# hellolijj/gpu-topology-on-k8s

Measured on AMD Instinct MI355X. Metric: RCCL all-reduce bus GB/s on scheduler-chosen k-GPU subset, k=1/2/4/8, higher is better.
Workload: dtype bf16

## Files before the change

csrc/common/stream_copy.h:

```cpp
#pragma once
#include <hip/hip_runtime.h>

#include <algorithm>
#include <cstddef>

namespace gtk {

typedef unsigned int u32x4 __attribute__((ext_vector_type(4)));

constexpr int kStreamBlock = 256;

template <int U>
__device__ __forceinline__ size_t stream_slices(const u32x4* __restrict__ src, u32x4* __restrict__ dst, size_t n_vec,
                                                size_t blk, size_t nblk) {
  const size_t tile = (size_t)kStreamBlock * U;
  const size_t n_tiles = n_vec / tile;
  const size_t per = (n_tiles + nblk - 1) / nblk;
  const size_t t0 = blk * per;
  const size_t t1 = std::min(n_tiles, t0 + per);
  for (size_t t = t0; t < t1; ++t) {
    const size_t base = t * tile + threadIdx.x;
    u32x4 r[U];
#pragma unroll
    for (int u = 0; u < U; ++u) r[u] = __builtin_nontemporal_load(src + base + (size_t)u * kStreamBlock);
#pragma unroll
    for (int u = 0; u < U; ++u) __builtin_nontemporal_store(r[u], dst + base + (size_t)u * kStreamBlock);
  }
  return n_tiles * tile;
}

__device__ __forceinline__ void stream_vec_tail(const u32x4* __restrict__ src, u32x4* __restrict__ dst, size_t n_vec,
                                                size_t first, size_t blk, size_t nblk) {
  for (size_t i = first + blk * kStreamBlock + threadIdx.x; i < n_vec; i += nblk * kStreamBlock) dst[i] = src[i];
}

}
```

csrc/rccl/rccl_core.h:

```cpp
#pragma once
#include <hip/hip_runtime.h>
#include <rccl/rccl.h>

#include <algorithm>
#include <cstdint>
#include <cstdlib>
#include <cstring>
#include <stdexcept>
#include <string>
#include <vector>

#include "self_copy.h"

#define RCCL_HIP_CHECK(expr)                                                                     \
  do {                                                                                           \
    hipError_t _e = (expr);                                                                      \
    if (_e != hipSuccess)                                                                        \
      throw std::runtime_error(std::string(#expr " failed: ") + hipGetErrorString(_e) + " at " + \
                               __FILE__ + ":" + std::to_string(__LINE__));                       \
  } while (0)

#define NCCL_CHECK(expr)                                                                          \
  do {                                                                                            \
    ncclResult_t _r = (expr);                                                                     \
    if (_r != ncclSuccess)                                                                        \
      throw std::runtime_error(std::string(#expr " failed: ") + ncclGetErrorString(_r) + " at " + \
                               __FILE__ + ":" + std::to_string(__LINE__));                        \
  } while (0)

namespace gtk {

inline ncclDataType_t parse_dtype(const std::string& s, size_t* elem) {
  if (s == "bf16" || s == "bfloat16") {
    *elem = 2;
    return ncclBfloat16;
  }
  if (s == "fp16" || s == "half" || s == "float16") {
    *elem = 2;
    return ncclFloat16;
  }
  if (s == "fp32" || s == "float" || s == "float32") {
    *elem = 4;
    return ncclFloat32;
  }
  throw std::invalid_argument("dtype must be bf16|fp16|fp32");
}

inline double bus_factor(int k) { return k > 1 ? 2.0 * (k - 1) / k : 0.0; }

__global__ void gtk_fill_kernel(void* buf, size_t count, int dtype_code, int rank) {
  const float scale = (float)(rank + 1);
  for (size_t i = (size_t)blockIdx.x * blockDim.x + threadIdx.x; i < count; i += (size_t)gridDim.x * blockDim.x) {
    float v = scale * (float)((i % 7) + 1);
    if (dtype_code == 0) {
      __bf16 b = (__bf16)v;
      reinterpret_cast<__bf16*>(buf)[i] = b;
    } else if (dtype_code == 1) {
      reinterpret_cast<_Float16*>(buf)[i] = (_Float16)v;
    } else {
      reinterpret_cast<float*>(buf)[i] = v;
    }
  }
}

__global__ void gtk_check_kernel(const void* buf, size_t count, int dtype_code, int nranks,
                                 unsigned long long* bad) {
  const float tri = (float)(nranks * (nranks + 1) / 2);
  unsigned long long local = 0;
  for (size_t i = (size_t)blockIdx.x * blockDim.x + threadIdx.x; i < count; i += (size_t)gridDim.x * blockDim.x) {
    float want = tri * (float)((i % 7) + 1);
    float got;
    if (dtype_code == 0)
      got = (float)reinterpret_cast<const __bf16*>(buf)[i];
    else if (dtype_code == 1)
      got = (float)reinterpret_cast<const _Float16*>(buf)[i];
    else
      got = reinterpret_cast<const float*>(buf)[i];
    local += (got != want);
  }
  if (local) atomicAdd(bad, local);
}

inline int dtype_code(ncclDataType_t t) { return t == ncclBfloat16 ? 0 : (t == ncclFloat16 ? 1 : 2); }
inline size_t elem_size(ncclDataType_t t) { return t == ncclFloat32 ? 4 : 2; }

struct RankState {
  int device = -1, rank = 0, nranks = 1;
  ncclComm_t comm = nullptr;
  hipStream_t stream = nullptr;
  void* send = nullptr;
  void* recv = nullptr;
  size_t cap_bytes = 0;
  bool self_copy = true;
  size_t self_copy_min = kSelfCopyMinBytes;
  int cus = 0, max_blocks = 0;

  void set_device() const { RCCL_HIP_CHECK(hipSetDevice(device)); }

  void configure() {
    const char* e = std::getenv("GTK_RCCL_SELF_COPY");
    self_copy = !(e && std::strcmp(e, "0") == 0);
    RCCL_HIP_CHECK(hipDeviceGetAttribute(&cus, hipDeviceAttributeMultiprocessorCount, device));
    max_blocks = std::max(1, cus) * kSelfCopyBlocksPerCU;
  }

  void ensure(size_t bytes) {
    set_device();
    if (!stream) RCCL_HIP_CHECK(hipStreamCreateWithFlags(&stream, hipStreamNonBlocking));
    if (bytes <= cap_bytes) return;
    if (send) RCCL_HIP_CHECK(hipFree(send));
    if (recv) RCCL_HIP_CHECK(hipFree(recv));
    send = recv = nullptr;
    RCCL_HIP_CHECK(hipMalloc(&send, bytes));
    RCCL_HIP_CHECK(hipMalloc(&recv, bytes));
    cap_bytes = bytes;
  }

  void fill(size_t count, ncclDataType_t t) {
    set_device();
    hipLaunchKernelGGL(gtk_fill_kernel, dim3(1024), dim3(256), 0, stream, send, count, dtype_code(t), rank);
    RCCL_HIP_CHECK(hipGetLastError());
  }

  unsigned long long check(size_t count, ncclDataType_t t, bool inplace) {
    set_device();
    unsigned long long* d_bad = nullptr;
    RCCL_HIP_CHECK(hipMalloc(&d_bad, sizeof(unsigned long long)));
    RCCL_HIP_CHECK(hipMemsetAsync(d_bad, 0, sizeof(unsigned long long), stream));
    hipLaunchKernelGGL(gtk_check_kernel, dim3(1024), dim3(256), 0, stream, inplace ? send : recv, count, dtype_code(t),
                       nranks, d_bad);
    RCCL_HIP_CHECK(hipGetLastError());
    unsigned long long bad = 0;
    RCCL_HIP_CHECK(hipMemcpyAsync(&bad, d_bad, sizeof(bad), hipMemcpyDeviceToHost, stream));
    RCCL_HIP_CHECK(hipStreamSynchronize(stream));
    RCCL_HIP_CHECK(hipFree(d_bad));
    return bad;
  }

  void allreduce(size_t count, ncclDataType_t t, bool inplace) {
    if (nranks == 1 && self_copy) {
      if (inplace) return;
      const size_t bytes = count * elem_size(t);
      if (bytes >= self_copy_min) {
        if (!max_blocks) throw std::logic_error("RankState::configure() was not called");
        hipLaunchKernelGGL(gtk_self_copy_kernel, dim3(self_copy_grid(bytes, max_blocks)), dim3(kSelfCopyBlock), 0, stream,
                           send, recv, bytes);
        RCCL_HIP_CHECK(hipGetLastError());
        return;
      }
    }
    NCCL_CHECK(ncclAllReduce(send, inplace ? send : recv, count, t, ncclSum, comm, stream));
  }

  void release() {
    if (comm) {
      (void)hipSetDevice(device);
      (void)ncclCommDestroy(comm);
      comm = nullptr;
    }
    if (send) (void)hipFree(send);
    if (recv) (void)hipFree(recv);
    send = recv = nullptr;
    cap_bytes = 0;
    if (stream) (void)hipStreamDestroy(stream);
    stream = nullptr;
  }
};

struct SweepPoint {
  size_t bytes = 0;
  size_t count = 0;
  double time_us = 0, algbw = 0, busbw = 0;
  unsigned long long wrong = 0;
};

class LocalGroup {
 public:
  explicit LocalGroup(const std::vector<int>& devs) : ranks_(devs.size()) {
    if (devs.empty()) throw std::invalid_argument("empty device list");
    std::vector<ncclComm_t> comms(devs.size());
    std::vector<int> dl(devs.begin(), devs.end());
    NCCL_CHECK(ncclCommInitAll(comms.data(), (int)devs.size(), dl.data()));
    for (size_t i = 0; i < devs.size(); ++i) {
      ranks_[i].device = devs[i];
      ranks_[i].rank = (int)i;
      ranks_[i].nranks = (int)devs.size();
      ranks_[i].comm = comms[i];
      ranks_[i].configure();
    }
  }
  ~LocalGroup() {
    for (auto& r : ranks_) r.release();
  }
  LocalGroup(const LocalGroup&) = delete;
  LocalGroup& operator=(const LocalGroup&) = delete;

  SweepPoint run(size_t bytes, const std::string& dtype, int iters, int warmup, bool inplace, bool check) {
    size_t elem = 0;
    ncclDataType_t t = parse_dtype(dtype, &elem);
    const size_t count = std::max<size_t>(1, bytes / elem);
    bytes = count * elem;
    for (auto& r : ranks_) r.ensure(bytes);
    SweepPoint p;
    p.bytes = bytes;
    p.count = count;
    if (check) {
      for (auto& r : ranks_) r.fill(count, t);
      launch_all(count, t, inplace);
      sync_all();
      for (auto& r : ranks_) p.wrong += r.check(count, t, inplace);
    }
    for (int i = 0; i < warmup; ++i) launch_all(count, t, inplace);
    sync_all();
    std::vector<hipEvent_t> e0(ranks_.size()), e1(ranks_.size());
    for (size_t i = 0; i < ranks_.size(); ++i) {
      ranks_[i].set_device();
      RCCL_HIP_CHECK(hipEventCreate(&e0[i]));
      RCCL_HIP_CHECK(hipEventCreate(&e1[i]));
      RCCL_HIP_CHECK(hipEventRecord(e0[i], ranks_[i].stream));
    }
    for (int i = 0; i < iters; ++i) launch_all(count, t, inplace);
    float worst = 0.f;
    for (size_t i = 0; i < ranks_.size(); ++i) {
      ranks_[i].set_device();
      RCCL_HIP_CHECK(hipEventRecord(e1[i], ranks_[i].stream));
    }
    for (size_t i = 0; i < ranks_.size(); ++i) {
      ranks_[i].set_device();
      RCCL_HIP_CHECK(hipEventSynchronize(e1[i]));
      float ms = 0.f;
      RCCL_HIP_CHECK(hipEventElapsedTime(&ms, e0[i], e1[i]));
      worst = std::max(worst, ms);
      (void)hipEventDestroy(e0[i]);
      (void)hipEventDestroy(e1[i]);
    }
    p.time_us = worst * 1e3 / std::max(1, iters);
    p.algbw = (double)bytes / (p.time_us * 1e-6) / 1e9;
    p.busbw = p.algbw * bus_factor((int)ranks_.size());
    return p;
  }

  size_t size() const { return ranks_.size(); }
  void set_self_copy(bool on) {
    for (auto& r : ranks_) r.self_copy = on;
  }

 private:
  void launch_all(size_t count, ncclDataType_t t, bool inplace) {
    NCCL_CHECK(ncclGroupStart());
    for (auto& r : ranks_) {
      r.set_device();
      r.allreduce(count, t, inplace);
    }
    NCCL_CHECK(ncclGroupEnd());
  }
  void sync_all() {
    for (auto& r : ranks_) {
      r.set_device();
      RCCL_HIP_CHECK(hipStreamSynchronize(r.stream));
    }
  }
  std::vector<RankState> ranks_;
};

inline std::vector<size_t> size_sweep(size_t min_bytes, size_t max_bytes, int factor) {
  std::vector<size_t> out;
  factor = std::max(2, factor);
  for (size_t b = std::max<size_t>(min_bytes, 4); b <= max_bytes; b *= (size_t)factor) {
    out.push_back(b);
    if (b > max_bytes / (size_t)factor) break;
  }
  return out;
}

}
```

csrc/rccl/rccl_module.hip:

```cpp
#include <pybind11/pybind11.h>
#include <pybind11/stl.h>

#include "rccl_core.h"

namespace py = pybind11;
using namespace gtk;

namespace {

class Comm {
 public:
  Comm(py::bytes uid, int nranks, int rank, int device, int min_ctas, int max_ctas) {
    std::string s = uid;
    if (s.size() != sizeof(ncclUniqueId)) throw std::invalid_argument("unique id must be NCCL_UNIQUE_ID_BYTES long");
    ncclUniqueId id;
    std::memcpy(&id, s.data(), sizeof(id));
    st_.device = device;
    st_.rank = rank;
    st_.nranks = nranks;
    py::gil_scoped_release nogil;
    st_.set_device();
    st_.configure();
    if (min_ctas > 0 || max_ctas > 0) {
      ncclConfig_t cfg = NCCL_CONFIG_INITIALIZER;
      if (min_ctas > 0) cfg.minCTAs = min_ctas;
      if (max_ctas > 0) cfg.maxCTAs = max_ctas;
      NCCL_CHECK(ncclCommInitRankConfig(&st_.comm, nranks, id, rank, &cfg));
    } else {
      NCCL_CHECK(ncclCommInitRank(&st_.comm, nranks, id, rank));
    }
    min_ctas_ = min_ctas;
    max_ctas_ = max_ctas;
    RCCL_HIP_CHECK(hipStreamCreateWithFlags(&st_.stream, hipStreamNonBlocking));
  }
  ~Comm() {
    drop_graph();
    st_.release();
  }

  void prepare(size_t bytes, const std::string& dtype) {
    drop_graph();
    t_ = parse_dtype(dtype, &elem_);
    count_ = std::max<size_t>(1, bytes / elem_);
    st_.ensure(count_ * elem_);
    st_.fill(count_, t_);
    RCCL_HIP_CHECK(hipStreamSynchronize(st_.stream));
  }

  void step(bool inplace) {
    if (!count_) throw std::runtime_error("prepare() first");
    st_.set_device();
    st_.allreduce(count_, t_, inplace);
  }

  void synchronize() {
    st_.set_device();
    RCCL_HIP_CHECK(hipStreamSynchronize(st_.stream));
  }

  unsigned long long check(bool inplace) {
    if (!count_) throw std::runtime_error("prepare() first");
    st_.fill(count_, t_);
    st_.allreduce(count_, t_, inplace);
    return st_.check(count_, t_, inplace);
  }

  void capture(int n, bool inplace) {
    if (!count_) throw std::runtime_error("prepare() first");
    if (n < 1) throw std::invalid_argument("capture needs n >= 1");
    drop_graph();
    st_.set_device();
    st_.allreduce(count_, t_, inplace);
    RCCL_HIP_CHECK(hipStreamSynchronize(st_.stream));
    hipGraph_t g = nullptr;
    RCCL_HIP_CHECK(hipStreamBeginCapture(st_.stream, hipStreamCaptureModeThreadLocal));
    try {
      for (int i = 0; i < n; ++i) st_.allreduce(count_, t_, inplace);
    } catch (...) {
      (void)hipStreamEndCapture(st_.stream, &g);
      if (g) (void)hipGraphDestroy(g);
      throw;
    }
    RCCL_HIP_CHECK(hipStreamEndCapture(st_.stream, &g));
    hipError_t e = hipGraphInstantiate(&exec_, g, nullptr, nullptr, 0);
    (void)hipGraphDestroy(g);
    if (e != hipSuccess) {
      exec_ = nullptr;
      throw std::runtime_error(std::string("hipGraphInstantiate failed: ") + hipGetErrorString(e));
    }
    graph_n_ = n;
  }

  void replay() {
    if (!exec_) throw std::runtime_error("capture() first");
    st_.set_device();
    RCCL_HIP_CHECK(hipGraphLaunch(exec_, st_.stream));
  }

  int graph_ops() const { return graph_n_; }

  unsigned long long verify() {
    if (!count_) throw std::runtime_error("prepare() first");
    return st_.check(count_, t_, false);
  }

  py::bytes read_result(size_t first, size_t n, bool inplace) {
    if (!count_ || !st_.send || !st_.recv) throw std::runtime_error("prepare() first");
    if (first > count_ || n > count_ - first) throw std::out_of_range("read_result: range outside the prepared buffer");
    std::string host(n * elem_, '\0');
    if (n) {
      py::gil_scoped_release nogil;
      st_.set_device();
      const char* src = static_cast<const char*>(inplace ? st_.send : st_.recv) + first * elem_;
      RCCL_HIP_CHECK(hipMemcpyAsync(&host[0], src, n * elem_, hipMemcpyDeviceToHost, st_.stream));
      RCCL_HIP_CHECK(hipStreamSynchronize(st_.stream));
    }
    return py::bytes(host);
  }

  size_t bytes() const { return count_ * elem_; }
  size_t count() const { return count_; }
  int rank() const { return st_.rank; }
  int nranks() const { return st_.nranks; }
  int device() const { return st_.device; }
  int min_ctas() const { return min_ctas_; }
  int max_ctas() const { return max_ctas_; }
  bool self_copy() const { return st_.self_copy; }
  void set_self_copy(bool on) {
    if (on != st_.self_copy) drop_graph();
    st_.self_copy = on;
  }
  size_t self_copy_min_bytes() const { return st_.self_copy_min; }
  void set_self_copy_min_bytes(size_t bytes) {
    if (bytes != st_.self_copy_min) drop_graph();
    st_.self_copy_min = bytes;
  }
  int self_copy_cus() const { return st_.cus; }
  int self_copy_max_blocks() const { return st_.max_blocks; }
  void destroy() {
    drop_graph();
    st_.release();
  }

 private:
  void drop_graph() {
    if (exec_) {
      (void)hipSetDevice(st_.device);
      (void)hipStreamSynchronize(st_.stream);
      (void)hipGraphExecDestroy(exec_);
    }
    exec_ = nullptr;
    graph_n_ = 0;
  }
  hipGraphExec_t exec_ = nullptr;
  int graph_n_ = 0;

  RankState st_;
  ncclDataType_t t_ = ncclBfloat16;
  size_t elem_ = 2, count_ = 0;
  int min_ctas_ = 0, max_ctas_ = 0;
};

py::bytes unique_id() {
  ncclUniqueId id;
  NCCL_CHECK(ncclGetUniqueId(&id));
  return py::bytes(reinterpret_cast<const char*>(&id), sizeof(id));
}

py::list local_sweep(const std::vector<int>& devs, const std::vector<size_t>& sizes, const std::string& dtype, int iters,
                     int warmup, bool inplace, bool check) {
  std::vector<SweepPoint> pts;
  {
    py::gil_scoped_release nogil;
    LocalGroup g(devs);
    for (size_t b : sizes) pts.push_back(g.run(b, dtype, iters, warmup, inplace, check));
  }
  py::list out;
  for (const auto& p : pts) {
    py::dict d;
    d["bytes"] = p.bytes;
    d["count"] = p.count;
    d["time_us"] = p.time_us;
    d["algbw_gbps"] = p.algbw;
    d["busbw_gbps"] = p.busbw;
    d["wrong"] = p.wrong;
    out.append(d);
  }
  return out;
}

int version() {
  int v = 0;
  NCCL_CHECK(ncclGetVersion(&v));
  return v;
}

}

PYBIND11_MODULE(_rccl, m) {
  m.doc() = "RCCL all-reduce placement validator (xGMI)";
  m.def("version", &version);
  m.def("unique_id", &unique_id);
  m.def("bus_factor", &bus_factor, py::arg("k"));
  m.def("size_sweep", &size_sweep, py::arg("min_bytes"), py::arg("max_bytes"), py::arg("factor") = 2);
  m.def("local_sweep", &local_sweep, py::arg("devs"), py::arg("sizes"), py::arg("dtype") = "bf16", py::arg("iters") = 20,
        py::arg("warmup") = 5, py::arg("inplace") = false, py::arg("check") = true);
  py::class_<Comm>(m, "Comm")
      .def(py::init<py::bytes, int, int, int, int, int>(), py::arg("uid"), py::arg("nranks"), py::arg("rank"),
           py::arg("device"), py::arg("min_ctas") = 0, py::arg("max_ctas") = 0)
      .def("prepare", &Comm::prepare, py::arg("bytes"), py::arg("dtype") = "bf16",
           py::call_guard<py::gil_scoped_release>())
      .def("step", &Comm::step, py::arg("inplace") = false, py::call_guard<py::gil_scoped_release>())
      .def("capture", &Comm::capture, py::arg("n"), py::arg("inplace") = false, py::call_guard<py::gil_scoped_release>())
      .def("replay", &Comm::replay, py::call_guard<py::gil_scoped_release>())
      .def_property_readonly("graph_ops", &Comm::graph_ops)
      .def("verify", &Comm::verify, py::call_guard<py::gil_scoped_release>())
      .def("synchronize", &Comm::synchronize, py::call_guard<py::gil_scoped_release>())
      .def("check", &Comm::check, py::arg("inplace") = false, py::call_guard<py::gil_scoped_release>())
      .def("destroy", &Comm::destroy, py::call_guard<py::gil_scoped_release>())
      .def("read_result", &Comm::read_result, py::arg("first"), py::arg("n"), py::arg("inplace") = false)
      .def_property_readonly("bytes", &Comm::bytes)
      .def_property_readonly("count", &Comm::count)
      .def_property_readonly("rank", &Comm::rank)
      .def_property_readonly("nranks", &Comm::nranks)
      .def_property_readonly("device", &Comm::device)
      .def_property_readonly("min_ctas", &Comm::min_ctas)
      .def_property_readonly("max_ctas", &Comm::max_ctas)
      .def_property("self_copy", &Comm::self_copy, &Comm::set_self_copy)
      .def_property("self_copy_min_bytes", &Comm::self_copy_min_bytes, &Comm::set_self_copy_min_bytes)
      .def_property_readonly("self_copy_cus", &Comm::self_copy_cus)
      .def_property_readonly("self_copy_max_blocks", &Comm::self_copy_max_blocks);
  m.attr("SELF_COPY_TILE_BYTES") = kSelfCopyTileBytes;
  m.attr("SELF_COPY_BLOCKS_PER_CU") = kSelfCopyBlocksPerCU;
  m.attr("SELF_COPY_MIN_BYTES") = kSelfCopyMinBytes;
}
```

csrc/rccl/self_copy.h:

```cpp
#pragma once
#include <hip/hip_runtime.h>

#include <algorithm>
#include <cstddef>
#include <cstdint>

#include "../common/stream_copy.h"

namespace gtk {

constexpr int kSelfCopyBlock = 256;
constexpr int kSelfCopyUnroll = 4;
constexpr int kSelfCopyBlocksPerCU = 8;
constexpr size_t kSelfCopyTileVec = (size_t)kSelfCopyBlock * kSelfCopyUnroll;
constexpr size_t kSelfCopyTileBytes = kSelfCopyTileVec * sizeof(u32x4);
static_assert(kSelfCopyBlock == kStreamBlock, "stream_copy.h indexes blocks of kStreamBlock threads");

constexpr size_t kSelfCopyMinBytes = (size_t)256 << 20;

__global__ __launch_bounds__(kSelfCopyBlock) void gtk_self_copy_kernel(const void* __restrict__ src_,
                                                                        void* __restrict__ dst_, size_t bytes) {
  const u32x4* __restrict__ src = static_cast<const u32x4*>(src_);
  u32x4* __restrict__ dst = static_cast<u32x4*>(dst_);
  const size_t n_vec = bytes / sizeof(u32x4);
  const size_t first = stream_slices<kSelfCopyUnroll>(src, dst, n_vec, blockIdx.x, gridDim.x);
  stream_vec_tail(src, dst, n_vec, first, blockIdx.x, gridDim.x);
  if (blockIdx.x == 0) {
    const size_t done = n_vec * sizeof(u32x4);
    const size_t units = (bytes - done) / sizeof(uint16_t);
    if (threadIdx.x < units) {
      const uint16_t* s = reinterpret_cast<const uint16_t*>(static_cast<const char*>(src_) + done);
      uint16_t* d = reinterpret_cast<uint16_t*>(static_cast<char*>(dst_) + done);
      d[threadIdx.x] = s[threadIdx.x];
    }
  }
}

inline unsigned self_copy_grid(size_t bytes, int max_blocks) {
  const size_t tiles = (bytes + kSelfCopyTileBytes - 1) / kSelfCopyTileBytes;
  return (unsigned)std::max<size_t>(1, std::min<size_t>(tiles, (size_t)max_blocks));
}

}
```

gpu_topology_on_k8s_amd/_native/build.py:

```python
from __future__ import annotations

import argparse
import concurrent.futures as cf
import os
import shlex
import subprocess
import sys
import sysconfig
from dataclasses import dataclass, field
from pathlib import Path
from typing import Dict, List, Optional

HERE = Path(__file__).resolve().parent
REPO = HERE.parent.parent
CSRC = REPO / "csrc"
ROCM = Path(os.environ.get("ROCM_PATH", "/opt/rocm"))
ARCH = os.environ.get("GTK_OFFLOAD_ARCH", "gfx950")
EXT = sysconfig.get_config_var("EXT_SUFFIX") or ".so"


def _py_includes() -> List[str]:
    import pybind11

    return [f"-I{sysconfig.get_paths()['include']}", f"-I{pybind11.get_include()}"]


def _torch_flags() -> List[str]:
    import torch
    from torch.utils import cpp_extension as ce

    inc = [f"-I{p}" for p in ce.include_paths()]
    libdir = str(Path(torch.__file__).parent / "lib")
    return inc + [
        "-D__HIP_PLATFORM_AMD__=1",
        "-DUSE_ROCM=1",
        "-DTORCH_EXTENSION_NAME=_fused",
        f"-D_GLIBCXX_USE_CXX11_ABI={int(torch._C._GLIBCXX_USE_CXX11_ABI)}",
        f"-L{libdir}",
        "-lc10",
        "-ltorch",
        "-ltorch_cpu",
        "-ltorch_python",
        "-lc10_hip",
        "-ltorch_hip",
        f"-Wl,-rpath,{libdir}",
    ]


@dataclass
class Target:
    name: str
    sources: List[Path]
    compiler: str
    out: Path
    extra: List[str] = field(default_factory=list)
    deps: List[Path] = field(default_factory=list)
    pybind: bool = True
    torch: bool = False
    shared: bool = True
    src_flags: Dict[str, List[str]] = field(default_factory=dict)

    def command(self) -> List[str]:
        if self.compiler == "hipcc":
            cmd = [str(ROCM / "bin" / "hipcc"), f"--offload-arch={ARCH}", "-O3", "-std=c++17"]
        else:
            cmd = ["g++", "-O3", "-std=c++17", "-Wall", "-Wno-unused-function"]
        if self.shared:
            cmd += ["-shared", "-fPIC", "-fvisibility=hidden"]
        cmd += [f"-I{ROCM / 'include'}", f"-I{CSRC}"]
        if self.pybind:
            cmd += _py_includes()
        cmd += [str(s) for s in self.sources]
        if self.torch:
            cmd += _torch_flags()
        cmd += self.extra
        cmd += ["-o", str(self.out)]
        return cmd

    def compile_flags(self) -> List[str]:
        cmd = [str(ROCM / "bin" / "hipcc"), f"--offload-arch={ARCH}", "-O3", "-std=c++17", "-fPIC", "-fvisibility=hidden",
               f"-I{ROCM / 'include'}", f"-I{CSRC}"]
        if self.pybind:
            cmd += _py_includes()
        if self.torch:
            cmd += [f for f in _torch_flags() if f.startswith(("-I", "-D"))]
        return cmd

    def link_flags(self) -> List[str]:
        flags = [f for f in _torch_flags() if not f.startswith(("-I", "-D"))] if self.torch else []
        return flags + [f for f in self.extra if not f.startswith(("-I", "-D"))]

    def up_to_date(self) -> bool:
        if not self.out.exists():
            return False
        t = self.out.stat().st_mtime
        inputs = list(self.sources) + list(self.deps) + [Path(__file__)]
        return all(p.stat().st_mtime <= t for p in inputs if p.exists())


def targets() -> List[Target]:
    rocm_lib = str(ROCM / "lib")
    stream_copy = CSRC / "common" / "stream_copy.h"
    return [
        Target("_topo", [CSRC / "topo" / "topo_reader.cpp"], "gxx", HERE / f"_topo{EXT}", ["-ldl"]),
        Target("topo_selftest", [CSRC / "topo" / "topo_selftest.cpp"], "gxx", HERE / "bin" / "topo_selftest",
               ["-g", "-O1", "-fsanitize=address,undefined", "-fno-sanitize-recover=undefined", "-fno-omit-frame-pointer",
                "-ldl"], deps=[CSRC / "topo" / "topo_reader.cpp"], pybind=False, shared=False),
        Target("fake_amdsmi", [CSRC / "topo" / "fake_amdsmi.cpp"], "gxx", HERE / "bin" / "libfake_amdsmi.so",
               ["-fvisibility=default"], pybind=False),
        Target("_placement", [CSRC / "placement" / "engine.cpp", CSRC / "placement" / "engine_module.cpp"], "gxx",
               HERE / f"_placement{EXT}", deps=[CSRC / "placement" / "engine.h"]),
        Target("engine_selftest", [CSRC / "placement" / "engine.cpp", CSRC / "placement" / "engine_selftest.cpp"], "gxx",
               HERE / "bin" / "engine_selftest", ["-g", "-O1", "-fsanitize=address,undefined", "-fno-omit-frame-pointer"],
               deps=[CSRC / "placement" / "engine.h"], pybind=False, shared=False),
        Target("_probe", [CSRC / "probe" / "probe.hip"], "hipcc", HERE / f"_probe{EXT}",
               deps=[stream_copy, CSRC / "probe" / "peer_allreduce.h", CSRC / "probe" / "chase_latency.h"]),
        Target("_rccl", [CSRC / "rccl" / "rccl_module.hip"], "hipcc", HERE / f"_rccl{EXT}",
               [f"-L{rocm_lib}", "-lrccl", f"-Wl,-rpath,{rocm_lib}"],
               deps=[CSRC / "rccl" / "rccl_core.h", CSRC / "rccl" / "self_copy.h", stream_copy]),
        Target("rccl_allreduce_bench", [CSRC / "rccl" / "rccl_allreduce_bench.hip"], "hipcc",
               HERE / "bin" / "rccl_allreduce_bench", [f"-L{rocm_lib}", "-lrccl", f"-Wl,-rpath,{rocm_lib}"],
               deps=[CSRC / "rccl" / "rccl_core.h", CSRC / "rccl" / "self_copy.h", stream_copy], pybind=False, shared=False),
        Target("vgpu_guard", [CSRC / "vgpu" / "vgpu_guard.cpp"], "gxx", HERE / "bin" / "libgtk_vgpu.so",
               ["-fvisibility=hidden", "-ldl", "-pthread"], pybind=False),
        Target("fake_hsa", [CSRC / "vgpu" / "fake_hsa.cpp"], "gxx", HERE / "bin" / "fake_hip" / "libhsa-runtime64.so",
               ["-fvisibility=default", "-pthread", "-Wl,-soname,libhsa-runtime64.so"], pybind=False),
        Target("fake_hip", [CSRC / "vgpu" / "fake_hip.cpp"], "gxx", HERE / "bin" / "fake_hip" / "libamdhip64.so",
               ["-fvisibility=default", f"-L{HERE / 'bin' / 'fake_hip'}", "-l:libhsa-runtime64.so", "-Wl,--disable-new-dtags", "-Wl,-rpath,$ORIGIN"],
               deps=[HERE / "bin" / "fake_hip" / "libhsa-runtime64.so"], pybind=False),
        Target("vgpu_selftest_tsan", [CSRC / "vgpu" / "vgpu_guard.cpp", CSRC / "vgpu" / "vgpu_selftest.cpp"], "gxx",
               HERE / "bin" / "vgpu_selftest_tsan",
               ["-g", "-O1", "-fsanitize=thread", "-pthread", "-ldl", f"-L{HERE / 'bin' / 'fake_hip'}", "-l:libamdhip64.so",
                "-l:libhsa-runtime64.so", "-Wl,--disable-new-dtags", f"-Wl,-rpath,{HERE / 'bin' / 'fake_hip'}"],
               deps=[HERE / "bin" / "fake_hip" / "libamdhip64.so"], pybind=False, shared=False),
        Target("vgpu_selftest_asan", [CSRC / "vgpu" / "vgpu_guard.cpp", CSRC / "vgpu" / "vgpu_selftest.cpp"], "gxx",
               HERE / "bin" / "vgpu_selftest_asan",
               ["-g", "-O1", "-fsanitize=address,undefined", "-fno-omit-frame-pointer", "-pthread", "-ldl",
                f"-L{HERE / 'bin' / 'fake_hip'}", "-l:libamdhip64.so", "-l:libhsa-runtime64.so", "-Wl,--disable-new-dtags",
                f"-Wl,-rpath,{HERE / 'bin' / 'fake_hip'}"],
               deps=[HERE / "bin" / "fake_hip" / "libamdhip64.so"], pybind=False, shared=False),
        Target("_fused", sorted((CSRC / "ops").glob("*.hip")), "hipcc", HERE / f"_fused{EXT}",
               deps=sorted((CSRC / "ops").glob("*.h")), pybind=True, torch=True,
               src_flags={"attention.hip": ["-mllvm", "-amdgpu-mfma-vgpr-form=1"]}),
    ]


OBJ = HERE / "obj"


def _run(cmd: List[str], what: str, verbose: bool) -> None:
    if verbose:
        print(" ".join(shlex.quote(c) for c in cmd), flush=True)
    p = subprocess.run(cmd, capture_output=True, text=True)
    if p.returncode != 0:
        raise RuntimeError(f"build of {what} failed ({p.returncode}):\n{' '.join(cmd)}\n{p.stdout}\n{p.stderr}")


def _build_objects(t: Target, force: bool, verbose: bool, jobs: int) -> str:
    odir = OBJ / t.name
    odir.mkdir(parents=True, exist_ok=True)
    dep_t = max([p.stat().st_mtime for p in list(t.deps) + [Path(__file__)] if p.exists()] or [0.0])
    flags = t.compile_flags()

    def one(src: Path) -> Path:
        obj = odir / (src.stem + ".o")
        if force or not obj.exists() or obj.stat().st_mtime < max(src.stat().st_mtime, dep_t):
            _run(flags + t.src_flags.get(src.name, []) + ["-c", str(src), "-o", str(obj)], f"{t.name}:{src.name}", verbose)
        return obj

    with cf.ThreadPoolExecutor(max_workers=max(1, min(jobs, len(t.sources)))) as ex:
        objs = list(ex.map(one, t.sources))
    if not force and t.out.exists() and all(o.stat().st_mtime <= t.out.stat().st_mtime for o in objs) and t.up_to_date():
        return f"ok   {t.name} (up to date)"
    t.out.parent.mkdir(parents=True, exist_ok=True)
    _run([str(ROCM / "bin" / "hipcc"), f"--offload-arch={ARCH}", "-shared", "-fPIC"] + [str(o) for o in objs]
         + t.link_flags() + ["-o", str(t.out)], t.name, verbose)
    return f"built {t.name} -> {t.out.relative_to(REPO)} ({len(objs)} objects)"


def build_one(t: Target, force: bool = False, verbose: bool = False, jobs: int = 4) -> str:
    missing = [s for s in t.sources if not s.exists()]
    if not t.sources or missing:
        return f"skip {t.name} (no sources)"
    if not force and t.up_to_date():
        return f"ok   {t.name} (up to date)"
    if t.compiler == "hipcc" and t.shared and len(t.sources) > 1:
        return _build_objects(t, force, verbose, jobs)
    t.out.parent.mkdir(parents=True, exist_ok=True)
    cmd = t.command()
    if verbose:
        print(" ".join(shlex.quote(c) for c in cmd), flush=True)
    p = subprocess.run(cmd, capture_output=True, text=True)
    if p.returncode != 0:
        raise RuntimeError(f"build of {t.name} failed ({p.returncode}):\n{' '.join(cmd)}\n{p.stdout}\n{p.stderr}")
    return f"built {t.name} -> {t.out.relative_to(REPO)}"


def build(force: bool = False, only: Optional[List[str]] = None, jobs: int = 4, verbose: bool = False) -> List[str]:
    ts = [t for t in targets() if not only or t.name in only]
    msgs: List[str] = []
    errors: List[str] = []
    producer = {t.out: t for t in targets()}

    def depth(t: Target) -> int:
        return 1 + max((depth(producer[d]) for d in t.deps if d in producer), default=-1)

    layers = [depth(t) for t in ts]
    waves = [[t for t, d in zip(ts, layers) if d == k] for k in range(max(layers, default=-1) + 1)]
    with cf.ThreadPoolExecutor(max_workers=max(1, jobs)) as ex:
        for wave in waves:
            futs = {ex.submit(build_one, t, force, verbose, jobs): t for t in wave}
            for f in cf.as_completed(futs):
                try:
                    msgs.append(f.result())
                except Exception as e:
                    errors.append(str(e))
    if errors:
        raise RuntimeError("\n\n".join(errors))
    return sorted(msgs)


def main(argv: Optional[List[str]] = None) -> int:
    ap = argparse.ArgumentParser(description=__doc__, formatter_class=argparse.RawDescriptionHelpFormatter)
    ap.add_argument("--force", action="store_true")
    ap.add_argument("--only", default="")
    ap.add_argument("-j", "--jobs", type=int, default=4)
    ap.add_argument("-v", "--verbose", action="store_true")
    a = ap.parse_args(argv)
    only = [s for s in a.only.split(",") if s] or None
    for m in build(a.force, only, a.jobs, a.verbose):
        print(m)
    return 0


if __name__ == "__main__":
    sys.exit(main())
```

Baseline: 2732.

## Add size-banded self-copy routing with grid-strided sweep kernel for single-rank copies

Adds a second single-rank copy kernel that walks tiles grid-strided (round*nblk+blk) instead of in contiguous per-block slices, with an optional look-ahead touch of a future tile. A band table now picks RCCL below 136 MiB, the sweep kernel up to about 1984 MiB, and the slice kernel above that. This lowers the self-copy cutoff from 256 MiB. It aims to improve DRAM access locality and to avoid RCCL overhead in the mid-size range, at the cost of extra size-tuned thresholds and runtime knobs.

```diff
diff --git a/csrc/common/stream_copy.h b/csrc/common/stream_copy.h
--- a/csrc/common/stream_copy.h
+++ b/csrc/common/stream_copy.h
@@ -3,6 +3,8 @@
 
 #include <algorithm>
 #include <cstddef>
+
+#include "stream_index.h"
 
 namespace gtk {
 
@@ -14,10 +16,9 @@
 __device__ __forceinline__ size_t stream_slices(const u32x4* __restrict__ src, u32x4* __restrict__ dst, size_t n_vec,
                                                 size_t blk, size_t nblk) {
   const size_t tile = (size_t)kStreamBlock * U;
-  const size_t n_tiles = n_vec / tile;
-  const size_t per = (n_tiles + nblk - 1) / nblk;
-  const size_t t0 = blk * per;
-  const size_t t1 = std::min(n_tiles, t0 + per);
+  const size_t n_tiles = stream_tiles(n_vec, tile);
+  const size_t t0 = slice_begin(n_tiles, blk, nblk);
+  const size_t t1 = slice_end(n_tiles, blk, nblk);
   for (size_t t = t0; t < t1; ++t) {
     const size_t base = t * tile + threadIdx.x;
     u32x4 r[U];
@@ -26,7 +27,34 @@
 #pragma unroll
     for (int u = 0; u < U; ++u) __builtin_nontemporal_store(r[u], dst + base + (size_t)u * kStreamBlock);
   }
-  return n_tiles * tile;
+  return stream_tail_first(n_vec, tile);
+}
+
+template <int U>
+__device__ __forceinline__ size_t stream_sweep(const u32x4* __restrict__ src, u32x4* __restrict__ dst, size_t n_vec,
+                                               size_t blk, size_t nblk, size_t ahead) {
+  const size_t tile = (size_t)kStreamBlock * U;
+  const size_t n_tiles = stream_tiles(n_vec, tile);
+  const size_t rounds = sweep_rounds(n_tiles, blk, nblk);
+  for (size_t rnd = 0; rnd < rounds; ++rnd) {
+    const size_t base = sweep_tile(blk, nblk, rnd) * tile + threadIdx.x;
+    u32x4 r[U];
+#pragma unroll
+    for (int u = 0; u < U; ++u) r[u] = __builtin_nontemporal_load(src + base + (size_t)u * kStreamBlock);
+    size_t touch = 0;
+    unsigned int ts = 0, td = 0;
+    if (sweep_touch(rounds, tile, blk, nblk, rnd, ahead, &touch) && threadIdx.x == 0) {
+      unsigned int lo = (unsigned int)touch;
+      asm volatile("" : "+v"(lo));
+      touch = (touch & ~(size_t)0xffffffffu) | lo;
+      ts = __builtin_nontemporal_load(reinterpret_cast<const unsigned int*>(src + touch));
+      td = __builtin_nontemporal_load(reinterpret_cast<const unsigned int*>(dst + touch));
+    }
+#pragma unroll
+    for (int u = 0; u < U; ++u) __builtin_nontemporal_store(r[u], dst + base + (size_t)u * kStreamBlock);
+    asm volatile("" ::"v"(ts), "v"(td));
+  }
+  return stream_tail_first(n_vec, tile);
 }
 
 __device__ __forceinline__ void stream_vec_tail(const u32x4* __restrict__ src, u32x4* __restrict__ dst, size_t n_vec,
diff --git a/csrc/common/stream_index.h b/csrc/common/stream_index.h
--- /dev/null
+++ b/csrc/common/stream_index.h
@@ -0,0 +1,47 @@
+#pragma once
+#include <cstddef>
+
+#if defined(__HIPCC__)
+#define GTK_STREAM_HD __host__ __device__
+#else
+#define GTK_STREAM_HD
+#endif
+
+namespace gtk {
+
+GTK_STREAM_HD inline size_t stream_tiles(size_t n_vec, size_t tile) { return n_vec / tile; }
+
+GTK_STREAM_HD inline size_t stream_tail_first(size_t n_vec, size_t tile) { return stream_tiles(n_vec, tile) * tile; }
+
+GTK_STREAM_HD inline size_t slice_per_block(size_t n_tiles, size_t nblk) { return (n_tiles + nblk - 1) / nblk; }
+
+GTK_STREAM_HD inline size_t slice_begin(size_t n_tiles, size_t blk, size_t nblk) {
+  return blk * slice_per_block(n_tiles, nblk);
+}
+GTK_STREAM_HD inline size_t slice_end(size_t n_tiles, size_t blk, size_t nblk) {
+  const size_t end = slice_begin(n_tiles, blk, nblk) + slice_per_block(n_tiles, nblk);
+  return end < n_tiles ? end : n_tiles;
+}
+
+GTK_STREAM_HD inline size_t slice_rounds(size_t n_tiles, size_t blk, size_t nblk) {
+  const size_t t0 = slice_begin(n_tiles, blk, nblk), t1 = slice_end(n_tiles, blk, nblk);
+  return t0 < t1 ? t1 - t0 : 0;
+}
+GTK_STREAM_HD inline size_t slice_tile(size_t n_tiles, size_t blk, size_t nblk, size_t round) {
+  return slice_begin(n_tiles, blk, nblk) + round;
+}
+
+GTK_STREAM_HD inline size_t sweep_rounds(size_t n_tiles, size_t blk, size_t nblk) {
+  return blk < n_tiles ? (n_tiles - blk + nblk - 1) / nblk : 0;
+}
+
+GTK_STREAM_HD inline size_t sweep_tile(size_t blk, size_t nblk, size_t round) { return round * nblk + blk; }
+
+GTK_STREAM_HD inline bool sweep_touch(size_t rounds, size_t tile, size_t blk, size_t nblk, size_t round, size_t ahead,
+                                      size_t* index) {
+  if (ahead == 0 || round + ahead >= rounds) return false;
+  *index = sweep_tile(blk, nblk, round + ahead) * tile;
+  return true;
+}
+
+}
diff --git a/csrc/rccl/rccl_core.h b/csrc/rccl/rccl_core.h
--- a/csrc/rccl/rccl_core.h
+++ b/csrc/rccl/rccl_core.h
@@ -91,8 +91,11 @@
   void* send = nullptr;
   void* recv = nullptr;
   size_t cap_bytes = 0;
+  enum Walk { walk_auto, walk_slice, walk_sweep };
   bool self_copy = true;
   size_t self_copy_min = kSelfCopyMinBytes;
+  Walk walk = walk_auto;
+  int ahead = 0;
   int cus = 0, max_blocks = 0;
 
   void set_device() const { RCCL_HIP_CHECK(hipSetDevice(device)); }
@@ -137,14 +140,28 @@
     return bad;
   }
 
+  SelfCopyPlan route(size_t bytes) const {
+    SelfCopyPlan p = self_copy_plan(bytes);
+    if (p.path == SelfCopyPath::rccl && bytes < self_copy_min) return p;
+    if (p.path == SelfCopyPath::rccl) p = {SelfCopyPath::slice, 0};
+    if (walk == walk_slice) p = {SelfCopyPath::slice, 0};
+    if (walk == walk_sweep) p = {SelfCopyPath::sweep, ahead};
+    return p;
+  }
+
   void allreduce(size_t count, ncclDataType_t t, bool inplace) {
     if (nranks == 1 && self_copy) {
       if (inplace) return;
       const size_t bytes = count * elem_size(t);
-      if (bytes >= self_copy_min) {
+      const SelfCopyPlan p = route(bytes);
+      if (p.path != SelfCopyPath::rccl) {
         if (!max_blocks) throw std::logic_error("RankState::configure() was not called");
-        hipLaunchKernelGGL(gtk_self_copy_kernel, dim3(self_copy_grid(bytes, max_blocks)), dim3(kSelfCopyBlock), 0, stream,
-                           send, recv, bytes);
+        const dim3 grid(self_copy_grid(bytes, max_blocks));
+        if (p.path == SelfCopyPath::sweep)
+          hipLaunchKernelGGL(gtk_self_copy_sweep_kernel, grid, dim3(kSelfCopyBlock), 0, stream, send, recv, bytes,
+                             (unsigned)p.ahead);
+        else
+          hipLaunchKernelGGL(gtk_self_copy_kernel, grid, dim3(kSelfCopyBlock), 0, stream, send, recv, bytes);
         RCCL_HIP_CHECK(hipGetLastError());
         return;
       }
diff --git a/csrc/rccl/rccl_module.hip b/csrc/rccl/rccl_module.hip
--- a/csrc/rccl/rccl_module.hip
+++ b/csrc/rccl/rccl_module.hip
@@ -137,6 +137,29 @@
   }
   int self_copy_cus() const { return st_.cus; }
   int self_copy_max_blocks() const { return st_.max_blocks; }
+  void set_self_copy_max_blocks(int n) {
+    if (n < 1) throw std::invalid_argument("self_copy_max_blocks must be at least 1");
+    if (n != st_.max_blocks) drop_graph();
+    st_.max_blocks = n;
+  }
+  std::string self_copy_walk() const {
+    return st_.walk == RankState::walk_auto ? "auto" : st_.walk == RankState::walk_slice ? "slice" : "sweep";
+  }
+  void set_self_copy_walk(const std::string& w) {
+    RankState::Walk v;
+    if (w == "auto") v = RankState::walk_auto;
+    else if (w == "slice") v = RankState::walk_slice;
+    else if (w == "sweep") v = RankState::walk_sweep;
+    else throw std::invalid_argument("self_copy_walk must be auto|slice|sweep");
+    if (v != st_.walk) drop_graph();
+    st_.walk = v;
+  }
+  int self_copy_ahead() const { return st_.ahead; }
+  void set_self_copy_ahead(int n) {
+    if (n < 0) throw std::invalid_argument("self_copy_ahead must be at least 0");
+    if (n != st_.ahead) drop_graph();
+    st_.ahead = n;
+  }
   void destroy() {
     drop_graph();
     st_.release();
@@ -184,6 +207,26 @@
     d["algbw_gbps"] = p.algbw;
     d["busbw_gbps"] = p.busbw;
     d["wrong"] = p.wrong;
+    out.append(d);
+  }
+  return out;
+}
+
+py::dict self_copy_plan_dict(size_t bytes) {
+  const SelfCopyPlan p = self_copy_plan(bytes);
+  py::dict d;
+  d["path"] = self_copy_path_name(p.path);
+  d["ahead"] = p.ahead;
+  return d;
+}
+
+py::list self_copy_bands() {
+  py::list out;
+  for (const SelfCopyBand& b : kSelfCopyBands) {
+    py::dict d;
+    d["from"] = b.from;
+    d["path"] = self_copy_path_name(b.plan.path);
+    d["ahead"] = b.plan.ahead;
     out.append(d);
   }
   return out;
@@ -229,7 +272,11 @@
       .def_property("self_copy", &Comm::self_copy, &Comm::set_self_copy)
       .def_property("self_copy_min_bytes", &Comm::self_copy_min_bytes, &Comm::set_self_copy_min_bytes)
       .def_property_readonly("self_copy_cus", &Comm::self_copy_cus)
-      .def_property_readonly("self_copy_max_blocks", &Comm::self_copy_max_blocks);
+      .def_property("self_copy_max_blocks", &Comm::self_copy_max_blocks, &Comm::set_self_copy_max_blocks)
+      .def_property("self_copy_walk", &Comm::self_copy_walk, &Comm::set_self_copy_walk)
+      .def_property("self_copy_ahead", &Comm::self_copy_ahead, &Comm::set_self_copy_ahead);
+  m.def("self_copy_plan", &self_copy_plan_dict, py::arg("bytes"));
+  m.def("self_copy_bands", &self_copy_bands);
   m.attr("SELF_COPY_TILE_BYTES") = kSelfCopyTileBytes;
   m.attr("SELF_COPY_BLOCKS_PER_CU") = kSelfCopyBlocksPerCU;
   m.attr("SELF_COPY_MIN_BYTES") = kSelfCopyMinBytes;
diff --git a/csrc/rccl/self_copy.h b/csrc/rccl/self_copy.h
--- a/csrc/rccl/self_copy.h
+++ b/csrc/rccl/self_copy.h
@@ -6,24 +6,18 @@
 #include <cstdint>
 
 #include "../common/stream_copy.h"
+#include "self_copy_plan.h"
 
 namespace gtk {
 
-constexpr int kSelfCopyBlock = 256;
-constexpr int kSelfCopyUnroll = 4;
-constexpr int kSelfCopyBlocksPerCU = 8;
-constexpr size_t kSelfCopyTileVec = (size_t)kSelfCopyBlock * kSelfCopyUnroll;
-constexpr size_t kSelfCopyTileBytes = kSelfCopyTileVec * sizeof(u32x4);
 static_assert(kSelfCopyBlock == kStreamBlock, "stream_copy.h indexes blocks of kStreamBlock threads");
+static_assert(kSelfCopyVecBytes == sizeof(u32x4), "the plan header counts the same 16-byte vectors");
 
-constexpr size_t kSelfCopyMinBytes = (size_t)256 << 20;
-
-__global__ __launch_bounds__(kSelfCopyBlock) void gtk_self_copy_kernel(const void* __restrict__ src_,
-                                                                        void* __restrict__ dst_, size_t bytes) {
+__device__ __forceinline__ void self_copy_tails(const void* __restrict__ src_, void* __restrict__ dst_, size_t bytes,
+                                                size_t first) {
   const u32x4* __restrict__ src = static_cast<const u32x4*>(src_);
   u32x4* __restrict__ dst = static_cast<u32x4*>(dst_);
   const size_t n_vec = bytes / sizeof(u32x4);
-  const size_t first = stream_slices<kSelfCopyUnroll>(src, dst, n_vec, blockIdx.x, gridDim.x);
   stream_vec_tail(src, dst, n_vec, first, blockIdx.x, gridDim.x);
   if (blockIdx.x == 0) {
     const size_t done = n_vec * sizeof(u32x4);
@@ -36,6 +30,21 @@
   }
 }
 
+__global__ __launch_bounds__(kSelfCopyBlock) void gtk_self_copy_kernel(const void* __restrict__ src_,
+                                                                        void* __restrict__ dst_, size_t bytes) {
+  const size_t first = stream_slices<kSelfCopyUnroll>(static_cast<const u32x4*>(src_), static_cast<u32x4*>(dst_),
+                                                      bytes / sizeof(u32x4), blockIdx.x, gridDim.x);
+  self_copy_tails(src_, dst_, bytes, first);
+}
+
+__global__ __launch_bounds__(kSelfCopyBlock) void gtk_self_copy_sweep_kernel(const void* __restrict__ src_,
+                                                                              void* __restrict__ dst_, size_t bytes,
+                                                                              unsigned ahead) {
+  const size_t first = stream_sweep<kSelfCopyUnroll>(static_cast<const u32x4*>(src_), static_cast<u32x4*>(dst_),
+                                                     bytes / sizeof(u32x4), blockIdx.x, gridDim.x, ahead);
+  self_copy_tails(src_, dst_, bytes, first);
+}
+
 inline unsigned self_copy_grid(size_t bytes, int max_blocks) {
   const size_t tiles = (bytes + kSelfCopyTileBytes - 1) / kSelfCopyTileBytes;
   return (unsigned)std::max<size_t>(1, std::min<size_t>(tiles, (size_t)max_blocks));
diff --git a/csrc/rccl/self_copy_plan.h b/csrc/rccl/self_copy_plan.h
--- /dev/null
+++ b/csrc/rccl/self_copy_plan.h
@@ -0,0 +1,62 @@
+#pragma once
+#include <cstddef>
+
+#include "../common/stream_index.h"
+
+namespace gtk {
+
+constexpr int kSelfCopyBlock = 256;
+constexpr int kSelfCopyUnroll = 4;
+constexpr int kSelfCopyBlocksPerCU = 8;
+constexpr size_t kSelfCopyVecBytes = 16;
+constexpr size_t kSelfCopyTileVec = (size_t)kSelfCopyBlock * kSelfCopyUnroll;
+constexpr size_t kSelfCopyTileBytes = kSelfCopyTileVec * kSelfCopyVecBytes;
+
+enum class SelfCopyPath { rccl, slice, sweep };
+struct SelfCopyPlan {
+  SelfCopyPath path;
+  int ahead;
+};
+struct SelfCopyBand {
+  size_t from;
+  SelfCopyPlan plan;
+};
+
+constexpr SelfCopyBand kSelfCopyBands[] = {
+    {0, {SelfCopyPath::rccl, 0}},
+    {(size_t)136 << 20, {SelfCopyPath::sweep, 0}},
+    {((size_t)1984 << 20) + 2, {SelfCopyPath::slice, 0}},
+};
+constexpr int kSelfCopyBandCount = (int)(sizeof(kSelfCopyBands) / sizeof(kSelfCopyBands[0]));
+
+constexpr SelfCopyPlan self_copy_plan(size_t bytes) {
+  SelfCopyPlan p = kSelfCopyBands[0].plan;
+  for (int i = 1; i < kSelfCopyBandCount && bytes >= kSelfCopyBands[i].from; ++i) p = kSelfCopyBands[i].plan;
+  return p;
+}
+
+constexpr size_t self_copy_kernels_only_from() {
+  size_t from = 0;
+  for (int i = 0; i < kSelfCopyBandCount; ++i)
+    if (kSelfCopyBands[i].plan.path == SelfCopyPath::rccl)
+      from = i + 1 < kSelfCopyBandCount ? kSelfCopyBands[i + 1].from : ~(size_t)0;
+  return from;
+}
+constexpr size_t kSelfCopyMinBytes = self_copy_kernels_only_from();
+
+constexpr bool self_copy_bands_ok() {
+  if (kSelfCopyBands[0].from != 0) return false;
+  for (int i = 1; i < kSelfCopyBandCount; ++i)
+    if (kSelfCopyBands[i].from <= kSelfCopyBands[i - 1].from) return false;
+  for (int i = 0; i < kSelfCopyBandCount; ++i)
+    if (kSelfCopyBands[i].plan.ahead < 0 || (kSelfCopyBands[i].plan.path != SelfCopyPath::sweep && kSelfCopyBands[i].plan.ahead))
+      return false;
+  return kSelfCopyBands[kSelfCopyBandCount - 1].plan.path != SelfCopyPath::rccl;
+}
+static_assert(self_copy_bands_ok(), "bands start at 0, ascend, carry `ahead` only on sweep bands, and end on a kernel");
+
+inline const char* self_copy_path_name(SelfCopyPath p) {
+  return p == SelfCopyPath::rccl ? "rccl" : p == SelfCopyPath::slice ? "slice" : "sweep";
+}
+
+}
diff --git a/csrc/rccl/self_copy_selftest.cpp b/csrc/rccl/self_copy_selftest.cpp
--- /dev/null
+++ b/csrc/rccl/self_copy_selftest.cpp
@@ -0,0 +1,130 @@
+#include <cstdio>
+#include <vector>
+
+#include "self_copy_plan.h"
+
+using namespace gtk;
+
+static int failures = 0;
+#define EXPECT(cond, ...)          \
+  do {                             \
+    if (!(cond)) {                 \
+      ++failures;                  \
+      std::printf("FAIL %s:%d: %s: ", __FILE__, __LINE__, #cond); \
+      std::printf(__VA_ARGS__);    \
+      std::printf("\n");           \
+    }                              \
+  } while (0)
+
+constexpr size_t T = 1024;
+constexpr size_t kBlock = 256;
+
+static void copy_tile(std::vector<int>& seen, size_t tile_index, size_t n_vec, size_t* beyond) {
+  for (size_t i = tile_index * T; i < tile_index * T + T; ++i) {
+    if (i >= n_vec) ++*beyond;
+    else ++seen[i];
+  }
+}
+
+static void copy_tail(std::vector<int>& seen, size_t first, size_t n_vec, size_t nblk) {
+  for (size_t blk = 0; blk < nblk; ++blk)
+    for (size_t thr = 0; thr < kBlock; ++thr)
+      for (size_t i = first + blk * kBlock + thr; i < n_vec; i += nblk * kBlock) ++seen[i];
+}
+
+static void check_walk(bool sweep, size_t n_vec, size_t nblk, size_t ahead) {
+  std::vector<int> seen(n_vec, 0);
+  size_t beyond = 0;
+  const size_t n_tiles = stream_tiles(n_vec, T);
+  for (size_t blk = 0; blk < nblk; ++blk) {
+    const size_t rounds = sweep ? sweep_rounds(n_tiles, blk, nblk) : slice_rounds(n_tiles, blk, nblk);
+    std::vector<size_t> tiles;
+    for (size_t r = 0; r < rounds; ++r) {
+      tiles.push_back(sweep ? sweep_tile(blk, nblk, r) : slice_tile(n_tiles, blk, nblk, r));
+      EXPECT(tiles.back() < n_tiles, "tile %zu of %zu (n_vec %zu nblk %zu blk %zu round %zu)", tiles.back(), n_tiles,
+             n_vec, nblk, blk, r);
+      copy_tile(seen, tiles.back(), n_vec, &beyond);
+    }
+    if (!sweep) continue;
+    for (size_t r = 0; r < rounds + 3; ++r) {
+      size_t idx = ~(size_t)0;
+      const bool on = sweep_touch(rounds, T, blk, nblk, r, ahead, &idx);
+      if (!on) {
+        EXPECT(ahead == 0 || r + ahead >= rounds, "no touch although round %zu + %zu exists (rounds %zu)", r, ahead, rounds);
+        continue;
+      }
+      EXPECT(ahead > 0 && r + ahead < rounds, "touch for a round that does not exist: %zu + %zu of %zu", r, ahead, rounds);
+      EXPECT(idx < n_vec, "touch index %zu >= n_vec %zu", idx, n_vec);
+      if (r + ahead < rounds)
+        EXPECT(idx == tiles[r + ahead] * T, "touch %zu is not the first index of tile %zu", idx, tiles[r + ahead]);
+    }
+  }
+  const size_t first = stream_tail_first(n_vec, T);
+  EXPECT(first <= n_vec && n_vec - first < T, "tail starts at %zu of %zu", first, n_vec);
+  copy_tail(seen, first, n_vec, nblk);
+  EXPECT(beyond == 0, "%zu indices at or past n_vec %zu (nblk %zu)", beyond, n_vec, nblk);
+  size_t wrong = 0;
+  for (size_t i = 0; i < n_vec; ++i) wrong += seen[i] != 1;
+  EXPECT(wrong == 0, "%zu of %zu indices not copied exactly once (%s, nblk %zu, ahead %zu)", wrong, n_vec,
+         sweep ? "sweep" : "slices", nblk, ahead);
+}
+
+static bool valid(SelfCopyPlan p) {
+  const bool known = p.path == SelfCopyPath::rccl || p.path == SelfCopyPath::slice || p.path == SelfCopyPath::sweep;
+  return known && p.ahead >= 0 && (p.path == SelfCopyPath::sweep || p.ahead == 0);
+}
+
+static bool same(SelfCopyPlan a, SelfCopyPlan b) { return a.path == b.path && a.ahead == b.ahead; }
+
+static void check_plan() {
+  for (int sh = 1; sh <= 35; ++sh) {
+    const size_t p2 = (size_t)1 << sh;
+    const size_t sizes[] = {p2 - 2, p2, p2 + 2};
+    for (size_t b : sizes) {
+      if (b < 2 || b > ((size_t)32 << 30)) continue;
+      EXPECT(valid(self_copy_plan(b)), "plan of %zu bytes", b);
+    }
+  }
+  EXPECT(kSelfCopyBands[0].from == 0, "first band starts at %zu", kSelfCopyBands[0].from);
+  bool kernels_only = true;
+  size_t expect_min = 0;
+  for (int i = 0; i < kSelfCopyBandCount; ++i) {
+    const SelfCopyBand& b = kSelfCopyBands[i];
+    EXPECT(same(self_copy_plan(b.from), b.plan), "band %d at its edge %zu", i, b.from);
+    EXPECT(same(self_copy_plan(b.from + 16 + 2), b.plan), "band %d just above its edge", i);
+    if (i) {
+      EXPECT(b.from > kSelfCopyBands[i - 1].from && b.from % 2 == 0, "band %d edge %zu", i, b.from);
+      EXPECT(same(self_copy_plan(b.from - 2), kSelfCopyBands[i - 1].plan), "band %d just below edge %zu", i - 1, b.from);
+    }
+    if (b.plan.path == SelfCopyPath::rccl) {
+      kernels_only = false;
+    } else if (!kernels_only) {
+      kernels_only = true;
+      expect_min = b.from;
+    }
+  }
+  EXPECT(kernels_only, "the last band must be a kernel's");
+  EXPECT(kSelfCopyMinBytes == expect_min, "kSelfCopyMinBytes %zu, expected %zu", kSelfCopyMinBytes, expect_min);
+  if (kSelfCopyMinBytes) EXPECT(self_copy_plan(kSelfCopyMinBytes - 2).path == SelfCopyPath::rccl, "just below the cutoff");
+  const size_t above[] = {kSelfCopyMinBytes, kSelfCopyMinBytes + 18, (size_t)2 << 30, (size_t)32 << 30};
+  for (size_t b : above) EXPECT(self_copy_plan(b).path != SelfCopyPath::rccl, "%zu bytes is at or above the cutoff", b);
+}
+
+int main() {
+  const size_t n_vecs[] = {0, 1, T - 1, T, T + 1, 3 * T, 3 * T + 1, 13 * T + 5, 64 * T};
+  const size_t nblks[] = {1, 2, 3, 8};
+  const size_t aheads[] = {0, 1, 2, 5};
+  int cases = 0;
+  for (size_t n_vec : n_vecs)
+    for (size_t nblk : nblks) {
+      check_walk(false, n_vec, nblk, 0);
+      ++cases;
+      for (size_t ahead : aheads) {
+        check_walk(true, n_vec, nblk, ahead);
+        ++cases;
+      }
+    }
+  check_plan();
+  std::printf("self_copy_selftest: %d walk cases, %d bands, %d failures\n", cases, kSelfCopyBandCount, failures);
+  return failures ? 1 : 0;
+}
diff --git a/gpu_topology_on_k8s_amd/_native/build.py b/gpu_topology_on_k8s_amd/_native/build.py
--- a/gpu_topology_on_k8s_amd/_native/build.py
+++ b/gpu_topology_on_k8s_amd/_native/build.py
@@ -101,6 +101,8 @@
 def targets() -> List[Target]:
     rocm_lib = str(ROCM / "lib")
     stream_copy = CSRC / "common" / "stream_copy.h"
+    stream_index = CSRC / "common" / "stream_index.h"
+    self_copy = [CSRC / "rccl" / "self_copy.h", CSRC / "rccl" / "self_copy_plan.h", stream_copy, stream_index]
     return [
         Target("_topo", [CSRC / "topo" / "topo_reader.cpp"], "gxx", HERE / f"_topo{EXT}", ["-ldl"]),
         Target("topo_selftest", [CSRC / "topo" / "topo_selftest.cpp"], "gxx", HERE / "bin" / "topo_selftest",
@@ -114,13 +116,16 @@
                HERE / "bin" / "engine_selftest", ["-g", "-O1", "-fsanitize=address,undefined", "-fno-omit-frame-pointer"],
                deps=[CSRC / "placement" / "engine.h"], pybind=False, shared=False),
         Target("_probe", [CSRC / "probe" / "probe.hip"], "hipcc", HERE / f"_probe{EXT}",
-               deps=[stream_copy, CSRC / "probe" / "peer_allreduce.h", CSRC / "probe" / "chase_latency.h"]),
+               deps=[stream_copy, stream_index, CSRC / "probe" / "peer_allreduce.h", CSRC / "probe" / "chase_latency.h"]),
         Target("_rccl", [CSRC / "rccl" / "rccl_module.hip"], "hipcc", HERE / f"_rccl{EXT}",
                [f"-L{rocm_lib}", "-lrccl", f"-Wl,-rpath,{rocm_lib}"],
-               deps=[CSRC / "rccl" / "rccl_core.h", CSRC / "rccl" / "self_copy.h", stream_copy]),
+               deps=[CSRC / "rccl" / "rccl_core.h"] + self_copy),
         Target("rccl_allreduce_bench", [CSRC / "rccl" / "rccl_allreduce_bench.hip"], "hipcc",
                HERE / "bin" / "rccl_allreduce_bench", [f"-L{rocm_lib}", "-lrccl", f"-Wl,-rpath,{rocm_lib}"],
-               deps=[CSRC / "rccl" / "rccl_core.h", CSRC / "rccl" / "self_copy.h", stream_copy], pybind=False, shared=False),
+               deps=[CSRC / "rccl" / "rccl_core.h"] + self_copy, pybind=False, shared=False),
+        Target("self_copy_selftest", [CSRC / "rccl" / "self_copy_selftest.cpp"], "gxx", HERE / "bin" / "self_copy_selftest",
+               ["-g", "-O1", "-fsanitize=address,undefined", "-fno-sanitize-recover=undefined", "-fno-omit-frame-pointer"],
+               deps=[CSRC / "rccl" / "self_copy_plan.h", stream_index], pybind=False, shared=False),
         Target("vgpu_guard", [CSRC / "vgpu" / "vgpu_guard.cpp"], "gxx", HERE / "bin" / "libgtk_vgpu.so",
                ["-fvisibility=hidden", "-ldl", "-pthread"], pybind=False),
         Target("fake_hsa", [CSRC / "vgpu" / "fake_hsa.cpp"], "gxx", HERE / "bin" / "fake_hip" / "libhsa-runtime64.so",
```

New measurement: 2730. About the same (-0.1%).
